# jamieapps101/Basic_Sparse_Matrix

Measured on AMD Instinct MI355X. Metric: CSR x dense SpMM effective GB/s (B_alg / step time); nnz/s, higher is better.
Workload: dtype f64

## Files before the change

### basic_sparse_matrix_amd/_lib.py

```python

from __future__ import annotations

import ctypes
import os
import threading

import numpy as np

try:
    import torch
except Exception:
    torch = None

LIB_PATH = os.environ.get("BSM_LIB_PATH") or os.path.join(os.path.dirname(os.path.abspath(__file__)), "lib",
                                                          "libbsm_hip.so")

BSM_F64, BSM_F32, BSM_I32, BSM_U32, BSM_I64, BSM_U64 = range(6)
DTYPE_CODES = {
    np.dtype(np.float64): BSM_F64,
    np.dtype(np.float32): BSM_F32,
    np.dtype(np.int32): BSM_I32,
    np.dtype(np.uint32): BSM_U32,
    np.dtype(np.int64): BSM_I64,
    np.dtype(np.uint64): BSM_U64,
}
CODE_DTYPES = {v: k for k, v in DTYPE_CODES.items()}

BSM_OK = 0
BSM_ERR_INVALID = 1
BSM_ERR_DIMENSIONS = 2
BSM_ERR_NON_SQUARE = 3
BSM_ERR_PANIC = 4
BSM_ERR_HIP = 5
BSM_ERR_OOM = 6
BSM_ERR_UNSUPPORTED = 7
BSM_TILED_ANY_PADDING = 1
BSM_ERR_NO_DEVICE = 8
BSM_ERR_OUT_OF_BOUNDS = 9
BSM_ERR_COMM = 10
BSM_UNIQUE_ID_BYTES = 128

ROWLEN_CONST, ROWLEN_UNIFORM, ROWLEN_BINOMIAL = 0, 1, 2
VAL_UNIFORM, VAL_SMALLINT = 0, 1


class DeviceUnavailable(RuntimeError):
    """The HIP library or a gfx950 device is not available (no CPU fallback)."""


class BsmError(RuntimeError):
    def __init__(self, code: int, msg: str):
        super().__init__(f"bsm error {code}: {msg}")
        self.code = code
        self.msg = msg


_u64 = ctypes.c_uint64
_u32 = ctypes.c_uint32
_int = ctypes.c_int
_vp = ctypes.c_void_p
_pp = ctypes.POINTER(ctypes.c_void_p)
_u64p = ctypes.POINTER(ctypes.c_uint64)

SIGNATURES = [
    ("bsm_api_version", _int, []),
    ("bsm_last_error", ctypes.c_char_p, []),
    ("bsm_stage_timing", _int, [_int]),
    ("bsm_stage_times", _int, [_int, ctypes.POINTER(_int), ctypes.c_char_p, ctypes.POINTER(ctypes.c_double)]),
    ("bsm_device_count", _int, [ctypes.POINTER(_int)]),
    ("bsm_set_device", _int, [_int]),
    ("bsm_csr_upload", _int, [_int, _u64, _u64, _u64, _vp, _vp, _vp, ctypes.POINTER(_vp)]),
    ("bsm_csr_from_inserts", _int, [_int, _u64, _u64, _u64, _vp, _vp, _vp, ctypes.POINTER(_vp)]),
    ("bsm_csr_from_coo", _int, [_int, _u64, _u64, _u64, _vp, _vp, _vp, ctypes.POINTER(_vp)]),
    ("bsm_csr_shape", _int, [_vp, _u64p, _u64p, _u64p, ctypes.POINTER(_int)]),
    ("bsm_csr_download", _int, [_vp, _vp, _vp, _vp]),
    ("bsm_host_register", _int, [_vp, _u64]),
    ("bsm_host_unregister", _int, [_vp]),
    ("bsm_csr_free", None, [_vp]),
    ("bsm_csr_mul_dense", _int, [_vp, _u64, _u64, _pp, ctypes.POINTER(_vp)]),
    ("bsm_csr_mul_vector", _int, [_vp, _vp, _u64, _vp, _u64]),
    ("bsm_csr_transpose", _int, [_vp, ctypes.POINTER(_vp)]),
    ("bsm_csr_add_sparse", _int, [_vp, _vp, ctypes.POINTER(_vp)]),
    ("bsm_csr_sub_sparse", _int, [_vp, _vp, ctypes.POINTER(_vp)]),
    ("bsm_csr_mul_sparse", _int, [_vp, _vp, ctypes.POINTER(_vp)]),
    ("bsm_csr_cholesky", _int, [_vp, ctypes.POINTER(_vp)]),
    ("bsm_forward_substitution", _int, [_vp, _u64, _u64, _pp, _pp]),
    ("bsm_backward_substitution", _int, [_vp, _u64, _u64, _pp, _pp]),
    ("bsm_solve", _int, [_vp, _u64, _u64, _pp, _pp]),
    ("bsm_solve_blocked", _int, [_vp, _u64, _u64, _pp, _pp]),
    ("bsm_solve_nd", _int, [_vp, _u64, _u64, _pp, _pp]),
    ("bsm_nd_factor_create", _int, [_vp, ctypes.POINTER(_vp)]),
    ("bsm_nd_factor_solve", _int, [_vp, _u64, _u64, _pp, _pp]),
    ("bsm_nd_factor_info", _int, [_vp, _u64p, ctypes.POINTER(_int), _u64p, _u64p]),
    ("bsm_nd_factor_perm", _int, [_vp, _vp]),
    ("bsm_nd_factor_export", _int, [_vp, ctypes.POINTER(_vp), ctypes.POINTER(_vp)]),
    ("bsm_nd_factor_refactor", _int, [_vp, _vp]),
    ("bsm_nd_factor_logdet", _int, [_vp, ctypes.POINTER(ctypes.c_double)]),
    ("bsm_nd_factor_solve_system", _int, [_vp, _int, _u64, _u64, _pp, _pp]),
    ("bsm_dev_nd_factor_solve", _int, [_vp, _int, _u64, _vp, _vp, _vp]),
    ("bsm_nd_factor_selinv", _int, [_vp, _vp, _u64, _vp, _vp, _vp]),
    ("bsm_dev_nd_factor_inv_diag", _int, [_vp, _vp, _vp]),
    ("bsm_nd_factor_free", None, [_vp]),
    ("bsm_nd_analyse", _int, [_u64, _vp, _vp, _u64, _vp, _vp, _u64, _u64p, _vp, _u64, _u64p]),
    ("bsm_nd_cache_clear", _int, []),
    ("bsm_nd_cache_info", _int, [_u64p, _u64p, _u64p, _u64p]),
    ("bsm_dev_gen_row_ptr", _int, [_u64, _u64, _u64, _u32, _int, _u32, _u32, _vp, _vp, _u64, _vp]),
    ("bsm_dev_gen_entries", _int, [_int, _u64, _u64, _u64, _u32, _int, _vp, _vp, _vp, _vp]),
    ("bsm_dev_gen_dense", _int, [_int, _u64, _u64, _u64, _u64, _int, _vp, _vp]),
    ("bsm_dev_gen_insert_stream", _int, [_int, _u64, _u64, _u64, _u64, _u64, _u64, _vp, _vp, _vp, _vp]),
    ("bsm_dev_csr_from_inserts", _int, [_int, _u64, _u64, _u64, _vp, _vp, _vp, ctypes.POINTER(_vp), _vp]),
    ("bsm_dev_scan_workspace_bytes", _u64, [_u64]),
    ("bsm_dev_spmm", _int, [_int, _u64, _u64, _u64, _vp, _vp, _vp, _u64, _vp, _vp, _vp, _vp]),
    ("bsm_csr_panel_cols", _int, [_vp, _u64p]),
    ("bsm_dev_spmm_panel_cols", _u64, [_int, _u64, _u64]),
    ("bsm_dev_spmm_plan_bytes", _u64, [_u64, _u64, _u64]),
    ("bsm_dev_spmm_plan", _int, [_u64, _u64, _vp, _vp, _u64, _vp, ctypes.POINTER(_int), _vp]),
    ("bsm_dev_spmm_panelled", _int, [_int, _u64, _u64, _u64, _vp, _vp, _vp, _u64, _vp, _vp, _vp, _u64, _vp, _vp]),
    ("bsm_dev_tiled_wanted", _int, [_int, _u64, _u64, _u64, _u64, _u64]),
    ("bsm_dev_tiled_create", _int, [_u64, _u64, _u64, _vp, _vp, _vp, _u64, _int, ctypes.POINTER(_vp), _vp]),
    ("bsm_dev_spmm_tiled", _int, [_vp, _vp, _vp, _vp, _vp]),
    ("bsm_tiled_info", _int, [_vp, _u64p, _u64p, _u64p]),
    ("bsm_tiled_destroy", None, [_vp]),
    ("bsm_csr_tiled", _int, [_vp, ctypes.POINTER(_int)]),
    ("bsm_dev_compact", _int, [_int, _u64, _u64, _vp, _vp, _vp, _vp, _vp, _vp, _u64, _vp]),
    ("bsm_multi_create", _int, [_int, ctypes.POINTER(_int), ctypes.POINTER(_vp)]),
    ("bsm_multi_unique_id", _int, [_vp]),
    ("bsm_multi_create_rank", _int, [_vp, _int, _int, _int, ctypes.POINTER(_vp)]),
    ("bsm_multi_create_external", _int, [_int, _int, _int, ctypes.POINTER(_vp)]),
    ("bsm_multi_is_external", _int, [_vp, ctypes.POINTER(_int)]),
    ("bsm_partition_rows", _int, [_vp, _u64, _u32, _vp]),
    ("bsm_multi_info", _int, [_vp, ctypes.POINTER(_int), ctypes.POINTER(_int), ctypes.POINTER(_int)]),
    ("bsm_multi_broadcast", _int, [_vp, _pp, _u64, _int]),
    ("bsm_multi_destroy", None, [_vp]),
    ("bsm_mcsr_upload", _int, [_vp, _int, _u64, _u64, _u64, _vp, _vp, _vp, _u32, ctypes.POINTER(_vp)]),
    ("bsm_mcsr_generate", _int, [_vp, _int, _u64, _u64, _u32, _int, _u32, _u32, _int, _u32, ctypes.POINTER(_vp)]),
    ("bsm_mcsr_info", _int, [_vp, _u64p, _u64p, _u64p, ctypes.POINTER(_u32), _u64p, _vp]),
    ("bsm_mcsr_prepare", _int, [_vp, _u64, _int, ctypes.POINTER(ctypes.c_double)]),
    ("bsm_mcsr_plan_info", _int, [_vp, ctypes.POINTER(_int), ctypes.POINTER(_int), _u64p, _u64p]),
    ("bsm_mcsr_mul_dense", _int, [_vp, _u64, _u64, _pp, ctypes.POINTER(_vp)]),
    ("bsm_mcsr_step", _int, [_vp, _pp]),
    ("bsm_mcsr_sync", _int, [_vp]),
    ("bsm_mcsr_step_times", _int, [_vp, _int, _int, ctypes.POINTER(_int), ctypes.POINTER(ctypes.c_double)]),
    ("bsm_mcsr_reset_times", None, [_vp]),
    ("bsm_mcsr_copy_y", _int, [_vp, _int, _vp, _vp]),
    ("bsm_mcsr_output", _int, [_vp, ctypes.POINTER(_vp)]),
    ("bsm_mcsr_compact", _int, [_vp]),
    ("bsm_mcsr_set_output_rank", _int, [_vp, _int]),
    ("bsm_mcsr_slot_read", _int, [_vp, _int, _u32, _u32, _vp, _vp]),
    ("bsm_mcsr_slot_write", _int, [_vp, _int, _u32, _u32, _vp, _vp]),
    ("bsm_mcsr_free", None, [_vp]),
]

_lock = threading.Lock()
_lib = None


def load(path: str = LIB_PATH) -> ctypes.CDLL:
    global _lib
    with _lock:
        if _lib is not None:
            return _lib
        if not os.path.exists(path):
            raise DeviceUnavailable(
                f"{path} is missing: build it with `python -c 'import __graft_entry__ as g; g.build()'`"
            )
        lib = ctypes.CDLL(path)
        for name, res, args in SIGNATURES:
            fn = getattr(lib, name)
            fn.restype = res
            fn.argtypes = args
        _lib = lib
        return lib


def stage_timing(on: bool = True) -> None:
    check(load().bsm_stage_timing(1 if on else 0))
# ... 138 lines not shown
```

### basic_sparse_matrix_amd/csrc/capi.hip

```cpp
#include <atomic>
#include <cstdarg>
#include <cstdlib>
#include <mutex>
#include <vector>

#include <algorithm>
#include <cstring>

#include "bsm_internal.hpp"

namespace bsm {

static thread_local std::string g_err;

void set_error(const char* fmt, ...) {
    char buf[1024];
    va_list ap;
    va_start(ap, fmt);
    vsnprintf(buf, sizeof(buf), fmt, ap);
    va_end(ap);
    g_err = buf;
}
const char* last_error() { return g_err.c_str(); }

// ... 1142 lines not shown
}

uint64_t bsm_dev_spmm_panel_cols(int dtype, uint64_t n_cols, uint64_t k) {
    return spmm_panel_cols(dtype, n_cols, k);
}

uint64_t bsm_dev_spmm_plan_bytes(uint64_t rows, uint64_t n_cols, uint64_t panel_cols) {
    return spmm_plan_bytes(rows, n_cols, panel_cols);
}

int bsm_dev_spmm_plan(uint64_t rows, uint64_t n_cols, const int64_t* row_ptr, const int32_t* col,
                      uint64_t panel_cols, int32_t* seg, int* usable, void* stream) {
    BSM_REQUIRE(row_ptr && usable && (spmm_plan_bytes(rows, n_cols, panel_cols) == 0 || seg),
                BSM_ERR_INVALID, "null argument");
    return spmm_plan(rows, n_cols, row_ptr, col, panel_cols, seg, usable,
                     static_cast<hipStream_t>(stream));
}

int bsm_dev_spmm_panelled(int dtype, uint64_t rows, uint64_t n_cols, uint64_t nnz,
                          const int64_t* row_ptr, const int32_t* col, const void* vals, uint64_t k,
                          const void* x, void* y, int32_t* row_nnz, uint64_t panel_cols,
                          const int32_t* seg, void* stream) {
    BSM_REQUIRE(row_ptr && (nnz == 0 || (col && vals)) && (k == 0 || (x && y)), BSM_ERR_INVALID,
                "null argument");
    if (k == 0) return BSM_OK;
    return spmm_panelled(dtype, rows, n_cols, nnz, row_ptr, col, vals, k, x, y, row_nnz, panel_cols,
                         seg, static_cast<hipStream_t>(stream));
}

int bsm_dev_tiled_wanted(int dtype, uint64_t rows, uint64_t n_cols, uint64_t nnz, uint64_t k,
                         uint64_t max_row_len) {
    return tiled_wanted(dtype, rows, n_cols, nnz, k, max_row_len) ? 1 : 0;
}

int bsm_dev_tiled_create(uint64_t rows, uint64_t n_cols, uint64_t nnz, const int64_t* row_ptr,
                         const int32_t* col, const double* vals, uint64_t k, int flags, bsm_tiled** out,
                         void* stream) {
    return tiled_create(BSM_F64, rows, n_cols, nnz, row_ptr, col, vals, k, flags, out, static_cast<hipStream_t>(stream));
}

int bsm_dev_spmm_tiled(const bsm_tiled* t, const double* x, double* y, int32_t* row_nnz, void* stream) {
    return tiled_spmm(t, x, y, row_nnz, false, static_cast<hipStream_t>(stream));
}

int bsm_tiled_info(const bsm_tiled* t, uint64_t* bytes, uint64_t* slots, uint64_t* panel_cols) {
    BSM_REQUIRE(t, BSM_ERR_INVALID, "null argument");
    const uint64_t n = (t->chunks + t->overread) * 64;
    if (bytes) *bytes = n * (t->meta_bytes + (t->dtype == BSM_F32 ? 4 : 8)) + ((uint64_t)t->nw * t->nb + 1) * 8;
    if (slots) *slots = t->chunks * 64;
    if (panel_cols) *panel_cols = 1ull << t->pshift;
    return BSM_OK;
}

void bsm_tiled_destroy(bsm_tiled* t) { tiled_destroy(t); }

int bsm_csr_tiled(const bsm_csr* m, int* in_use) {
    BSM_REQUIRE(m && in_use, BSM_ERR_INVALID, "null argument");
    std::lock_guard<std::mutex> lock(m->plan_mu);
    *in_use = m->tiled ? 1 : 0;
    return BSM_OK;
}

int bsm_dev_compact(int dtype, uint64_t rows, uint64_t k, const void* y, const int32_t* row_nnz,
                    int64_t* out_row_ptr, int32_t* out_col, void* out_vals, void* workspace,
                    uint64_t workspace_bytes, void* stream) {
    BSM_REQUIRE(row_nnz && out_row_ptr, BSM_ERR_INVALID, "null argument");
    hipStream_t s = static_cast<hipStream_t>(stream);
    BSM_TRY(exclusive_scan_i32_to_i64(row_nnz, out_row_ptr, rows, workspace, workspace_bytes, s));
    return compact_dispatch(dtype, rows, k, y, out_row_ptr, out_col, out_vals, s);
}

}
```

### basic_sparse_matrix_amd/csrc/kernels_tiled.hip

```cpp
#include "bsm_internal.hpp"

#include <cstdlib>
#include <type_traits>
#include <utility>
#include <vector>


namespace bsm {
namespace {

constexpr int WAVE = 64;
constexpr int CHUNK = 64;
constexpr int PHASES = 6;
constexpr int OVERREAD = 4;
constexpr uint32_t DONE = 0xffffffffu;
constexpr uint32_t RW_MAX = 155;
constexpr uint32_t RW_MAX_F32 = 255;
constexpr uint32_t PSHIFT = 12;
constexpr uint32_t PACE_PCT = 3;

__device__ __forceinline__ uint64_t lanemask_lt(int lane) {
    return lane == 0 ? 0ull : (~0ull >> (64 - lane));
}
__device__ __forceinline__ uint32_t wave_min_u32(uint32_t v) {
#pragma unroll
    for (int off = 1; off < WAVE; off <<= 1) v = min(v, (uint32_t)__shfl_xor((int)v, off, WAVE));
    return v;
}

template <bool WRITE, int SLOTS, typename V, typename M = uint32_t>
__global__ __launch_bounds__(256) void tiled_layout(uint64_t rows, uint64_t n_cols, double pace, uint32_t rbits,
                                                    uint32_t pad, const int64_t* __restrict__ rp,
                                                    const int32_t* __restrict__ col,
                                                    const V* __restrict__ vals, uint32_t nw,
                                                    uint32_t rpw, uint32_t nb, uint32_t rw, uint32_t pshift,
                                                    int32_t* __restrict__ counts,
                                                    const int64_t* __restrict__ offs,
                                                    M* __restrict__ meta, V* __restrict__ val) {
    const int lane = threadIdx.x & (WAVE - 1);
    const uint64_t task = (uint64_t)blockIdx.x * (blockDim.x / WAVE) + threadIdx.x / WAVE;
    if (task >= (uint64_t)nw * nb) return;
    const uint64_t gw = task / nb, b = task % nb;
    const uint64_t w0 = gw * rpw;
    const uint64_t wend = min<uint64_t>(rows, w0 + rpw);
    const uint64_t r0 = w0 + b * rw;
    int64_t cur[SLOTS], end[SLOTS];
    uint32_t h[SLOTS];
#pragma unroll
    for (int j = 0; j < SLOTS; ++j) {
        const uint32_t s = lane + WAVE * j;
        const bool live = s < rw && r0 + s < wend;
        cur[j] = live ? rp[r0 + s] : 0;
        end[j] = live ? rp[r0 + s + 1] : 0;
        h[j] = cur[j] < end[j] ? (uint32_t)col[cur[j]] >> pshift : DONE;
    }
    const bool any = r0 < wend;
    const int64_t t0 = any ? rp[r0] : 0, t1 = any ? rp[min<uint64_t>(r0 + rw, wend)] : 0;
    const double np = (double)(((n_cols - 1) >> pshift) + 1);
    const double inv_r = t1 > t0 ? (double)CHUNK * np / ((double)(t1 - t0) * pace) : 1e30;
    int64_t c = WRITE ? offs[task] : 0;
    int64_t n = 0;
    for (;;) {
        bool sel[SLOTS];
        int pos[SLOTS];
#pragma unroll
        for (int j = 0; j < SLOTS; ++j) {
            sel[j] = false;
            pos[j] = 0;
        }
        int taken = 0;
        const double pm = (double)n * inv_r;
        const uint32_t pmax = pm >= 4.0e9 ? DONE - 1 : (uint32_t)pm;
        bool done = false;
        while (taken < CHUNK) {
            uint32_t m = DONE;
#pragma unroll
            for (int j = 0; j < SLOTS; ++j) m = min(m, sel[j] ? DONE : h[j]);
            m = wave_min_u32(m);
            if (m == DONE) {
                done = taken == 0;
                break;
            }
            if (m > pmax) break;
            int before = 0;
#pragma unroll
            for (int j = 0; j < SLOTS; ++j) {
                const bool cand = !sel[j] && h[j] == m;
                const uint64_t bal = __ballot(cand);
                const int rank = before + __popcll(bal & lanemask_lt(lane));
                if (cand && taken + rank < CHUNK) {
                    sel[j] = true;
                    pos[j] = taken + rank;
                }
                before += __popcll(bal);
            }
            taken = min(taken + before, CHUNK);
        }
        if (done) break;
#pragma unroll
        for (int j = 0; j < SLOTS; ++j) {
            if (sel[j]) {
                const int64_t e = cur[j];
                if (WRITE) {
                    meta[c * CHUNK + pos[j]] = ((M)(uint32_t)col[e] << rbits) | (M)(lane + WAVE * j);
                    val[c * CHUNK + pos[j]] = vals[e];
                }
                cur[j] = e + 1;
                h[j] = cur[j] < end[j] ? (uint32_t)col[cur[j]] >> pshift : DONE;
            }
        }
        if (WRITE && lane >= taken) {
            meta[c * CHUNK + lane] = (M)rw;
            val[c * CHUNK + lane] = (V)0;
        }
        ++c;
        ++n;
    }
    const int64_t padded = (n + pad - 1) / pad * pad;
    if (WRITE) {
        for (int64_t p = n; p < padded; ++p, ++c) {
            meta[c * CHUNK + lane] = (M)rw;
            val[c * CHUNK + lane] = (V)0;
        }
    } else if (lane == 0) {
        counts[task] = (int32_t)padded;
    }
}

template <typename T> struct Vec2;
template <> struct Vec2<double> { using type = double2; };
struct F2 {
    uint64_t u;
};
template <> struct Vec2<float> { using type = F2; };
__device__ __forceinline__ double lo_of(const double2& v) { return v.x; }
__device__ __forceinline__ double hi_of(const double2& v) { return v.y; }
__device__ __forceinline__ float lo_of(const F2& v) { return __uint_as_float((uint32_t)v.u); }
__device__ __forceinline__ float hi_of(const F2& v) { return __uint_as_float((uint32_t)(v.u >> 32)); }
__device__ __forceinline__ double2 make_v2(double a, double b) { return make_double2(a, b); }
__device__ __forceinline__ F2 make_v2(float a, float b) {
    return F2{((uint64_t)__float_as_uint(b) << 32) | (uint64_t)__float_as_uint(a)};
}
template <typename T> using vec2_t = typename Vec2<T>::type;

template <typename T = double, typename M = uint32_t>
struct Idx {
    M mi;
    T vi;
};
template <typename T, typename M>
__device__ __forceinline__ void load_idx(Idx<T, M>& c, const M* __restrict__ meta, const T* __restrict__ val,
                                         int64_t chunk, int lane) {
    c.mi = meta[chunk * CHUNK + lane];
    c.vi = val[chunk * CHUNK + lane];
}
template <int I, typename T>
__device__ __forceinline__ uint32_t bm(const Idx<T, uint32_t>& c) {
    return (uint32_t)__builtin_amdgcn_update_dpp(0, (int)c.mi, 0x150 + I, 0xf, 0xf, false);
}
template <int I, typename T>
__device__ __forceinline__ uint64_t bm(const Idx<T, uint64_t>& c) {
    const uint32_t lo = (uint32_t)__builtin_amdgcn_update_dpp(0, (int)(uint32_t)c.mi, 0x150 + I, 0xf, 0xf, false);
// ... 259 lines not shown
    BSM_REQUIRE(k == 32 || k == 1, BSM_ERR_UNSUPPORTED, "tiled: k must be 32 or 1");
    BSM_REQUIRE(dtype == BSM_F64 || dtype == BSM_F32, BSM_ERR_UNSUPPORTED, "tiled: f64 or f32 only");
    const bool f32 = dtype == BSM_F32;
    const size_t es = f32 ? 4 : 8;
    const bool wide = k == 32 && n_cols >= (1ull << 24);
    const size_t mb = wide ? 8 : 4;
    const uint32_t rbits = k == 1 ? K1_RBITS : 8;
    BSM_REQUIRE(k == 32 ? n_cols <= 0x7fffffffull : n_cols < (1ull << (32 - rbits)), BSM_ERR_UNSUPPORTED,
                "tiled: columns must be < 2^%u", k == 32 ? 31u : 32 - rbits);
    *out = nullptr;
    int dev = 0;
    BSM_TRY(current_device(&dev));
    int cus = 0;
    BSM_HIP_TRY(hipDeviceGetAttribute(&cus, hipDeviceAttributeMultiprocessorCount, dev));
    if (s && cus > 0) {
        std::vector<uint32_t> mk((size_t)(cus + 31) / 32, 0u);
        if (hipExtStreamGetCUMask(s, (uint32_t)mk.size(), mk.data()) == hipSuccess) {
            int n = 0;
            for (int i = 0; i < cus; ++i) n += (mk[i / 32] >> (i % 32)) & 1u;
            if (n > 0 && n < cus) cus = n;
        } else {
            (void)hipGetLastError();
        }
    }
    const uint32_t wpc = k == 1 ? K1_WAVES_PER_CU : 4u;
    const uint32_t nw_env = env_u32("BSM_TILED_WAVES", wpc * (uint32_t)cus);
    const uint32_t nw = nw_env;
    const uint32_t k1_stage = env_u32("BSM_TILED_K1_STAGE", K1_STAGE_DEFAULT) == 8 ? 8u : 4u;
    const uint32_t rw_cap =
        k == 1 ? K1_RW_MAX : (f32 ? RW_MAX_F32 : RW_MAX);
    uint32_t rw_max = env_u32("BSM_TILED_RW", rw_cap);
    rw_max = rw_max < 8u ? 8u : (rw_max > rw_cap ? rw_cap : rw_max);
    const uint32_t pshift = env_u32("BSM_TILED_PSHIFT", k == 1 ? K1_PSHIFT : PSHIFT);
    const double pace = 1.0 + env_u32("BSM_TILED_PACE_PCT", PACE_PCT) / 100.0;
    const uint32_t pad = k == 1 ? 1u : PHASES;
    const uint32_t overread = k == 1 ? 2 * k1_stage : OVERREAD;
    BSM_REQUIRE(nw >= wpc && nw % wpc == 0 && pshift < 32, BSM_ERR_INVALID, "tiled: bad geometry");
    const uint64_t rpw64 = (rows + nw - 1) / nw;
    BSM_REQUIRE(rpw64 < (1ull << 31), BSM_ERR_UNSUPPORTED, "tiled: too many rows per wave");
    const uint32_t rpw = rpw64 ? (uint32_t)rpw64 : 1u;
    const uint32_t nb = (rpw + rw_max - 1) / rw_max;
    const uint32_t rw = (rpw + nb - 1) / nb;
    const uint64_t tasks = (uint64_t)nw * nb;

    DBuf counts, offs, ws;
    BSM_TRY(counts.alloc(tasks * sizeof(int32_t)));
    BSM_TRY(offs.alloc((tasks + 1) * sizeof(int64_t)));
    const uint64_t grid = (tasks + 3) / 4;
    auto layout = [&](auto write_tag, int32_t* cnt, const int64_t* of, void* me, void* va) -> int {
        constexpr bool W = decltype(write_tag)::value;
        auto go = [&]<typename V, typename MT>(V*, MT*) {
            if (k == 1)
                tiled_layout<W, (K1_RW_MAX + 1) / WAVE, V, MT><<<dim3((unsigned)grid), 256, 0, s>>>(
                    rows, n_cols, pace, rbits, pad, rp, col, static_cast<const V*>(vals), nw, rpw, nb, rw, pshift,
                    cnt, of, static_cast<MT*>(me), static_cast<V*>(va));
            else if (rw_cap > 192)
                tiled_layout<W, 4, V, MT><<<dim3((unsigned)grid), 256, 0, s>>>(
                    rows, n_cols, pace, rbits, pad, rp, col, static_cast<const V*>(vals), nw, rpw, nb, rw, pshift,
                    cnt, of, static_cast<MT*>(me), static_cast<V*>(va));
            else
                tiled_layout<W, 3, V, MT><<<dim3((unsigned)grid), 256, 0, s>>>(
                    rows, n_cols, pace, rbits, pad, rp, col, static_cast<const V*>(vals), nw, rpw, nb, rw, pshift,
                    cnt, of, static_cast<MT*>(me), static_cast<V*>(va));
        };
        if (f32 && wide) go((float*)nullptr, (uint64_t*)nullptr);
        else if (f32) go((float*)nullptr, (uint32_t*)nullptr);
        else if (wide) go((double*)nullptr, (uint64_t*)nullptr);
        else go((double*)nullptr, (uint32_t*)nullptr);
        BSM_HIP_TRY(hipGetLastError());
        return BSM_OK;
    };
    auto t_phase = host_now();
    auto phase_end = [&](double* acc) -> int {
        if (!pt) return BSM_OK;
        BSM_HIP_TRY(hipStreamSynchronize(s));
        *acc += ms_since(t_phase);
        t_phase = host_now();
        return BSM_OK;
    };
    BSM_TRY(layout(std::false_type{}, counts.as<int32_t>(), nullptr, nullptr, nullptr));
    BSM_TRY(phase_end(pt ? &pt->count_ms : nullptr));
    const uint64_t wsb = scan_workspace_bytes(tasks);
    BSM_TRY(ws.alloc(wsb));
    BSM_TRY(exclusive_scan_i32_to_i64(counts.as<int32_t>(), offs.as<int64_t>(), tasks, ws.p, wsb, s));
    int64_t total = 0;
    BSM_HIP_TRY(read_dev(&total, offs.as<int64_t>() + tasks, sizeof(total), s));
    BSM_TRY(phase_end(pt ? &pt->scan_ms : nullptr));
    BSM_REQUIRE((flags & BSM_TILED_ANY_PADDING) ||
                    (uint64_t)total * CHUNK <= nnz + nnz / 4 + tasks * pad * CHUNK + (uint64_t)CHUNK * 64,
                BSM_ERR_UNSUPPORTED, "tiled: %lld chunks for %llu entries (rows too uneven)", (long long)total,
                (unsigned long long)nnz);
    const uint64_t slots = ((uint64_t)total + overread) * CHUNK;
    size_t free_b = 0, total_b = 0;
    BSM_HIP_TRY(hipMemGetInfo(&free_b, &total_b));
    BSM_REQUIRE(slots * (mb + es) + (256ull << 20) + reserve < free_b, BSM_ERR_OOM,
                "tiled: %llu MB stream (+%llu MB reserved) does not fit", (unsigned long long)(slots * (mb + es) >> 20),
                (unsigned long long)(reserve >> 20));
    DBuf meta, val, bar;
    BSM_TRY(bar.alloc(8 * BAR_STRIDE * sizeof(unsigned)));
    BSM_TRY(meta.alloc(slots * mb));
    BSM_TRY(val.alloc(slots * es));
    BSM_TRY(phase_end(pt ? &pt->alloc_ms : nullptr));
    BSM_TRY(layout(std::true_type{}, nullptr, offs.as<int64_t>(), meta.p, val.p));
    BSM_HIP_TRY(hipMemsetAsync(static_cast<char*>(meta.p) + (uint64_t)total * CHUNK * mb, 0, overread * CHUNK * mb, s));
    BSM_HIP_TRY(hipMemsetAsync(static_cast<char*>(val.p) + (uint64_t)total * CHUNK * es, 0, overread * CHUNK * es, s));
    BSM_HIP_TRY(hipStreamSynchronize(s));
    BSM_TRY(phase_end(pt ? &pt->write_ms : nullptr));
    auto* t = new bsm_tiled;
    t->device = dev;
    t->dtype = dtype;
    t->k = k;
    t->rows = rows;
    t->n_cols = n_cols;
    t->nnz = nnz;
    t->nw = nw;
// ... 85 lines not shown
```

### basic_sparse_matrix_amd/device.py

```python

from __future__ import annotations

import ctypes
from dataclasses import dataclass

import numpy as np
import torch

from . import _lib

TORCH_DT = {
    np.dtype(np.float64): torch.float64,
    np.dtype(np.float32): torch.float32,
    np.dtype(np.int32): torch.int32,
    np.dtype(np.uint32): torch.uint32,
    np.dtype(np.int64): torch.int64,
    np.dtype(np.uint64): torch.uint64,
}


def _stream(stream=None) -> int:
    s = stream if stream is not None else torch.cuda.current_stream()
    return s.cuda_stream

# ... 53 lines not shown
            self.panel_cols, self.seg = w, seg
        return self.panel_cols

    def plan_tiled(self, k: int, force: bool = False) -> "TiledPlan | None":
        lib = _lib.require_device()
        self.tiled = None
        if self.dtype != np.float64 or k not in (1, 32) or self.nnz == 0:
            return None
        if not force:
            max_len = int((self.row_ptr[1:] - self.row_ptr[:-1]).max().item()) if self.rows else 0
            if not lib.bsm_dev_tiled_wanted(_lib.DTYPE_CODES[self.dtype], self.rows, self.n_cols, self.nnz, k,
                                            max_len):
                return None
        h = ctypes.c_void_p()
        rc = lib.bsm_dev_tiled_create(self.rows, self.n_cols, self.nnz, _p(self.row_ptr), _p(self.col),
                                      _p(self.vals), k, _lib.BSM_TILED_ANY_PADDING if force else 0,
                                      ctypes.byref(h), _stream())
        if rc in (_lib.BSM_ERR_UNSUPPORTED, _lib.BSM_ERR_OOM):
            return None
        _lib.check(rc)
        self.tiled = TiledPlan(h.value, k)
        return self.tiled

    def spmm(self, x: torch.Tensor, y: torch.Tensor, row_nnz: torch.Tensor | None = None, stream=None) -> None:
        lib = _lib.load()
        k = x.shape[1] if x.dim() == 2 else 1
        if self.tiled is not None and k == self.tiled.k:
            _lib.check(lib.bsm_dev_spmm_tiled(self.tiled.handle, _p(x), _p(y),
                                              _p(row_nnz) if row_nnz is not None else 0, _stream(stream)))
            return
        if self.seg is not None:
            _lib.check(lib.bsm_dev_spmm_panelled(_lib.DTYPE_CODES[self.dtype], self.rows, self.n_cols, self.nnz,
                                                 _p(self.row_ptr), _p(self.col), _p(self.vals), k, _p(x), _p(y),
                                                 _p(row_nnz) if row_nnz is not None else 0, self.panel_cols,
                                                 _p(self.seg), _stream(stream)))
            return
        _lib.check(lib.bsm_dev_spmm(_lib.DTYPE_CODES[self.dtype], self.rows, self.n_cols, self.nnz, _p(self.row_ptr),
                                    _p(self.col), _p(self.vals), k, _p(x), _p(y),
                                    _p(row_nnz) if row_nnz is not None else 0, _stream(stream)))


class TiledPlan:

    def __init__(self, handle: int, k: int = 32):
        self.handle = handle
        self.k = k

    def info(self) -> dict:
        lib = _lib.load()
        b, sl, pc = ctypes.c_uint64(), ctypes.c_uint64(), ctypes.c_uint64()
        _lib.check(lib.bsm_tiled_info(self.handle, ctypes.byref(b), ctypes.byref(sl), ctypes.byref(pc)))
        return {"bytes": b.value, "slots": sl.value, "panel_cols": pc.value}

    def __del__(self):
        if getattr(self, "handle", None) and _lib._lib is not None:
            _lib._lib.bsm_tiled_destroy(self.handle)
            self.handle = None


def gen_dense(seed, row0, n, k, value_kind=_lib.VAL_UNIFORM, dtype=np.float64, device="cuda") -> torch.Tensor:
    lib = _lib.require_device()
    dt = np.dtype(dtype)
    x = torch.empty((n, k), dtype=TORCH_DT[dt], device=device)
    _lib.check(lib.bsm_dev_gen_dense(_lib.DTYPE_CODES[dt], seed, row0, n, k, value_kind, _p(x), _stream()))
    return x


def nd_factor_solve(factor, b: torch.Tensor, out: torch.Tensor | None = None, *, system: str = "A",
                    stream=None) -> torch.Tensor:
    from .solver import nd_system_code
    from .sparse import _raise_for

    code = nd_system_code(system)
    want = TORCH_DT[np.dtype(factor.dtype)]
    out = torch.empty_like(b) if out is None else out
    for name, t in (("b", b), ("out", out)):
        if t.dtype != want:
            raise TypeError(f"nd_factor_solve: {name} is {t.dtype}, the factor is {factor.dtype}")
        if not t.is_cuda:
            raise ValueError(f"nd_factor_solve: {name} is not on the device")
        if t.dim() not in (1, 2) or t.shape[0] != factor.n or not t.is_contiguous():
            raise ValueError(f"nd_factor_solve: {name} must be contiguous, ({factor.n},) or ({factor.n}, k), "
                             f"got {tuple(t.shape)}")
    if out.shape != b.shape or out.device != b.device:
        raise ValueError(f"nd_factor_solve: out is {tuple(out.shape)} on {out.device}, b {tuple(b.shape)} on {b.device}")
    k = b.shape[1] if b.dim() == 2 else 1
    _raise_for(_lib.require_device().bsm_dev_nd_factor_solve(factor._h(), code, k, _p(b), _p(out), _stream(stream)))
    return out


def nd_factor_inv_diag(factor, out: torch.Tensor | None = None, *, stream=None) -> torch.Tensor:
    from .sparse import _raise_for

    h = factor._h()
    want = TORCH_DT[np.dtype(factor.dtype)]
    out = torch.empty((factor.n,), dtype=want, device="cuda") if out is None else out
    if out.dtype != want:
        raise TypeError(f"nd_factor_inv_diag: out is {out.dtype}, the factor is {factor.dtype}")
    if not out.is_cuda:
        raise ValueError("nd_factor_inv_diag: out is not on the device")
    if out.dim() != 1 or out.shape[0] != factor.n or not out.is_contiguous():
        raise ValueError(f"nd_factor_inv_diag: out must be contiguous, ({factor.n},), got {tuple(out.shape)}")
    _raise_for(_lib.require_device().bsm_dev_nd_factor_inv_diag(h, _p(out), _stream(stream)))
    return out


class Compactor:

    def __init__(self, rows: int, k: int, dtype, device="cuda"):
        lib = _lib.load()
# ... 41 lines not shown
```

### include/bsm.h

```cpp
#ifndef BSM_H
#define BSM_H

#include <stdint.h>

#ifdef __cplusplus
extern "C" {
#endif

#define BSM_API_VERSION 1

typedef enum bsm_dtype {
    BSM_F64 = 0,
    BSM_F32 = 1,
    BSM_I32 = 2,
    BSM_U32 = 3,
    BSM_I64 = 4,
    BSM_U64 = 5
} bsm_dtype;

typedef enum bsm_status {
    BSM_OK = 0,
    BSM_ERR_INVALID = 1,
    BSM_ERR_DIMENSIONS = 2,
    BSM_ERR_NON_SQUARE = 3,
// ... 60 lines not shown
int bsm_nd_factor_export(const bsm_nd_factor* f, bsm_csr** l, bsm_csr** l_star);
int bsm_nd_factor_refactor(bsm_nd_factor* f, const bsm_csr* a);
int bsm_nd_factor_logdet(const bsm_nd_factor* f, double* logdet);
int bsm_nd_factor_solve_system(const bsm_nd_factor* f, int system, uint64_t k, uint64_t n,
                               const void* const* b_cols, void* const* x_cols);
int bsm_dev_nd_factor_solve(const bsm_nd_factor* f, int system, uint64_t k, const void* b, void* x,
                            void* stream);
int bsm_nd_factor_selinv(const bsm_nd_factor* f, void* diag, uint64_t nq, const uint64_t* rows,
                         const uint64_t* cols, void* vals);
int bsm_dev_nd_factor_inv_diag(const bsm_nd_factor* f, void* diag, void* stream);
void bsm_nd_factor_free(bsm_nd_factor* f);
int bsm_nd_cache_clear(void);
int bsm_nd_cache_info(uint64_t* entries, uint64_t* kept_bytes, uint64_t* hits, uint64_t* misses);
int bsm_nd_analyse(uint64_t n, const uint64_t* row_ptr, const uint64_t* col_idx, uint64_t leaf,
                   int64_t* perm, int64_t* nodes, uint64_t cap, uint64_t* n_nodes, int64_t* st,
                   uint64_t st_cap, uint64_t* st_len);

int bsm_dev_gen_row_ptr(uint64_t seed, uint64_t row0, uint64_t rows, uint32_t n_cols,
                        int rowlen_kind, uint32_t a, uint32_t b, int64_t* row_ptr,
                        void* workspace, uint64_t workspace_bytes, void* stream);
int bsm_dev_gen_entries(int dtype, uint64_t seed, uint64_t row0, uint64_t rows,
                        uint32_t n_cols, int value_kind, const int64_t* row_ptr,
                        int32_t* col, void* vals, void* stream);
int bsm_dev_gen_insert_stream(int dtype, uint64_t seed, uint64_t i0, uint64_t n, uint64_t rows,
                              uint64_t cols, uint64_t vmod, uint64_t* row, uint64_t* col, void* vals,
                              void* stream);
int bsm_dev_csr_from_inserts(int dtype, uint64_t rows, uint64_t cols, uint64_t n, const uint64_t* row,
                             const uint64_t* col, const void* vals, bsm_csr** out, void* stream);
int bsm_dev_gen_dense(int dtype, uint64_t seed, uint64_t row0, uint64_t n, uint64_t k,
                      int value_kind, void* x, void* stream);
uint64_t bsm_dev_scan_workspace_bytes(uint64_t n);
int bsm_dev_spmm(int dtype, uint64_t rows, uint64_t n_cols, uint64_t nnz,
                 const int64_t* row_ptr, const int32_t* col, const void* vals, uint64_t k,
                 const void* x, void* y, int32_t* row_nnz, void* stream);
int bsm_csr_panel_cols(const bsm_csr* m, uint64_t* panel_cols);
uint64_t bsm_dev_spmm_panel_cols(int dtype, uint64_t n_cols, uint64_t k);
uint64_t bsm_dev_spmm_plan_bytes(uint64_t rows, uint64_t n_cols, uint64_t panel_cols);
int bsm_dev_spmm_plan(uint64_t rows, uint64_t n_cols, const int64_t* row_ptr, const int32_t* col,
                      uint64_t panel_cols, int32_t* seg, int* usable, void* stream);
int bsm_dev_spmm_panelled(int dtype, uint64_t rows, uint64_t n_cols, uint64_t nnz,
                          const int64_t* row_ptr, const int32_t* col, const void* vals, uint64_t k,
                          const void* x, void* y, int32_t* row_nnz, uint64_t panel_cols,
                          const int32_t* seg, void* stream);
typedef struct bsm_tiled bsm_tiled;
#define BSM_TILED_ANY_PADDING 1
int bsm_dev_tiled_wanted(int dtype, uint64_t rows, uint64_t n_cols, uint64_t nnz, uint64_t k,
                         uint64_t max_row_len);
int bsm_dev_tiled_create(uint64_t rows, uint64_t n_cols, uint64_t nnz, const int64_t* row_ptr,
                         const int32_t* col, const double* vals, uint64_t k, int flags,
                         bsm_tiled** out, void* stream);
int bsm_dev_spmm_tiled(const bsm_tiled* t, const double* x, double* y, int32_t* row_nnz,
                       void* stream);
int bsm_tiled_info(const bsm_tiled* t, uint64_t* bytes, uint64_t* slots, uint64_t* panel_cols);
int bsm_csr_tiled(const bsm_csr* m, int* in_use);
void bsm_tiled_destroy(bsm_tiled* t);
int bsm_dev_compact(int dtype, uint64_t rows, uint64_t k, const void* y,
                    const int32_t* row_nnz, int64_t* out_row_ptr, int32_t* out_col,
                    void* out_vals, void* workspace, uint64_t workspace_bytes, void* stream);

typedef struct bsm_multi bsm_multi;
typedef struct bsm_mcsr bsm_mcsr;
#define BSM_UNIQUE_ID_BYTES 128
int bsm_multi_create(int n_gpus, const int* devices, bsm_multi** out);
int bsm_multi_unique_id(void* id);
int bsm_multi_create_rank(const void* id, int world, int rank, int device, bsm_multi** out);
int bsm_multi_create_external(int world, int rank, int device, bsm_multi** out);
int bsm_multi_is_external(const bsm_multi* ctx, int* external);
int bsm_partition_rows(const uint64_t* row_ptr, uint64_t rows, uint32_t pieces, uint64_t* bounds);
int bsm_multi_info(const bsm_multi* ctx, int* world, int* n_local, int* first_rank);
int bsm_multi_broadcast(bsm_multi* ctx, void* const* bufs, uint64_t bytes, int root);
void bsm_multi_destroy(bsm_multi* ctx);

int bsm_mcsr_upload(bsm_multi* ctx, int dtype, uint64_t rows, uint64_t cols, uint64_t nnz,
                    const uint64_t* row_ptr, const uint64_t* col_idx, const void* vals, uint32_t chunks,
                    bsm_mcsr** out);
int bsm_mcsr_generate(bsm_multi* ctx, int dtype, uint64_t seed, uint64_t rows, uint32_t n_cols, int rowlen_kind,
                      uint32_t a, uint32_t b, int value_kind, uint32_t chunks, bsm_mcsr** out);
int bsm_mcsr_info(const bsm_mcsr* m, uint64_t* rows, uint64_t* cols, uint64_t* nnz, uint32_t* pieces,
                  uint64_t* piece_rows, uint64_t* bounds);
int bsm_mcsr_prepare(bsm_mcsr* m, uint64_t k, int schedule, double* plan_ms);
int bsm_mcsr_plan_info(const bsm_mcsr* m, int* tiled_pieces, int* local_pieces, uint64_t* copy_bytes,
                       uint64_t* panel_cols);
int bsm_mcsr_mul_dense(bsm_mcsr* m, uint64_t k, uint64_t x_rows, const void* const* x_cols, bsm_csr** out);
int bsm_mcsr_step(bsm_mcsr* m, const void* const* x_dev);
int bsm_mcsr_sync(bsm_mcsr* m);
int bsm_mcsr_step_times(bsm_mcsr* m, int local, int max, int* n, double* ms);
void bsm_mcsr_reset_times(bsm_mcsr* m);
int bsm_mcsr_copy_y(const bsm_mcsr* m, int local, void* y, int32_t* row_nnz);
int bsm_mcsr_output(const bsm_mcsr* m, bsm_csr** out);
int bsm_mcsr_set_output_rank(bsm_mcsr* m, int rank);
int bsm_mcsr_compact(bsm_mcsr* m);
int bsm_mcsr_slot_read(const bsm_mcsr* m, int local, uint32_t first, uint32_t n, void* y, int32_t* row_nnz);
int bsm_mcsr_slot_write(bsm_mcsr* m, int local, uint32_t first, uint32_t n, const void* y, const int32_t* row_nnz);
void bsm_mcsr_free(bsm_mcsr* m);

#ifdef __cplusplus
}
#endif

#endif
```

Before: 698.2.

## Speed up tiled layout build with DPP wave-min and windowed vector loads

The tiled_layout kernel that builds the tiled SpMM format now does its wave-wide minimum with DPP row operations plus readlane instead of a shuffle-xor loop. For small slot counts it also reads column indices and values through 32-byte aligned vector windows kept in registers, rather than issuing a scalar global load per element. The selection loop is rewritten to be branch-free. New geometry and download APIs expose the tiled buffers, presumably for verification. The cost is more register pressure from the per-slot windows, and the change only helps if layout construction falls inside the timed step.

```diff
diff --git a/basic_sparse_matrix_amd/_lib.py b/basic_sparse_matrix_amd/_lib.py
--- a/basic_sparse_matrix_amd/_lib.py
+++ b/basic_sparse_matrix_amd/_lib.py
@@ -61,6 +61,7 @@
 _vp = ctypes.c_void_p
 _pp = ctypes.POINTER(ctypes.c_void_p)
 _u64p = ctypes.POINTER(ctypes.c_uint64)
+_u32p = ctypes.POINTER(ctypes.c_uint32)
 
 SIGNATURES = [
     ("bsm_api_version", _int, []),
@@ -120,8 +121,11 @@
     ("bsm_dev_tiled_create", _int, [_u64, _u64, _u64, _vp, _vp, _vp, _u64, _int, ctypes.POINTER(_vp), _vp]),
     ("bsm_dev_spmm_tiled", _int, [_vp, _vp, _vp, _vp, _vp]),
     ("bsm_tiled_info", _int, [_vp, _u64p, _u64p, _u64p]),
+    ("bsm_tiled_geometry", _int, [_vp, _u64p, _u64p, _u32p, _u32p, _u32p, _u32p]),
+    ("bsm_tiled_download", _int, [_vp, _vp, _vp, _vp]),
     ("bsm_tiled_destroy", None, [_vp]),
     ("bsm_csr_tiled", _int, [_vp, ctypes.POINTER(_int)]),
+    ("bsm_csr_tiled_copy", _int, [_vp, ctypes.POINTER(_vp)]),
     ("bsm_dev_compact", _int, [_int, _u64, _u64, _vp, _vp, _vp, _vp, _vp, _vp, _u64, _vp]),
     ("bsm_multi_create", _int, [_int, ctypes.POINTER(_int), ctypes.POINTER(_vp)]),
     ("bsm_multi_unique_id", _int, [_vp]),
diff --git a/basic_sparse_matrix_amd/csrc/capi.hip b/basic_sparse_matrix_amd/csrc/capi.hip
--- a/basic_sparse_matrix_amd/csrc/capi.hip
+++ b/basic_sparse_matrix_amd/csrc/capi.hip
@@ -1218,12 +1218,40 @@
     return BSM_OK;
 }
 
+int bsm_tiled_geometry(const bsm_tiled* t, uint64_t* tasks, uint64_t* chunks, uint32_t* overread,
+                       uint32_t* meta_bytes, uint32_t* val_bytes, uint32_t* rw) {
+    BSM_REQUIRE(t, BSM_ERR_INVALID, "null argument");
+    if (tasks) *tasks = (uint64_t)t->nw * t->nb;
+    if (chunks) *chunks = t->chunks;
+    if (overread) *overread = t->overread;
+    if (meta_bytes) *meta_bytes = t->meta_bytes;
+    if (val_bytes) *val_bytes = t->dtype == BSM_F32 ? 4 : 8;
+    if (rw) *rw = t->rw;
+    return BSM_OK;
+}
+
+int bsm_tiled_download(const bsm_tiled* t, int64_t* offs, void* meta, void* val) {
+    BSM_REQUIRE(t, BSM_ERR_INVALID, "null argument");
+    const uint64_t n = (t->chunks + t->overread) * 64;
+    if (offs) BSM_HIP_TRY(hipMemcpy(offs, t->offs, ((uint64_t)t->nw * t->nb + 1) * sizeof(int64_t), hipMemcpyDeviceToHost));
+    if (meta) BSM_HIP_TRY(hipMemcpy(meta, t->meta, n * t->meta_bytes, hipMemcpyDeviceToHost));
+    if (val) BSM_HIP_TRY(hipMemcpy(val, t->val, n * (t->dtype == BSM_F32 ? 4 : 8), hipMemcpyDeviceToHost));
+    return BSM_OK;
+}
+
 void bsm_tiled_destroy(bsm_tiled* t) { tiled_destroy(t); }
 
 int bsm_csr_tiled(const bsm_csr* m, int* in_use) {
     BSM_REQUIRE(m && in_use, BSM_ERR_INVALID, "null argument");
     std::lock_guard<std::mutex> lock(m->plan_mu);
     *in_use = m->tiled ? 1 : 0;
+    return BSM_OK;
+}
+
+int bsm_csr_tiled_copy(const bsm_csr* m, const bsm_tiled** out) {
+    BSM_REQUIRE(m && out, BSM_ERR_INVALID, "null argument");
+    std::lock_guard<std::mutex> lock(m->plan_mu);
+    *out = m->tiled;
     return BSM_OK;
 }
 
diff --git a/basic_sparse_matrix_amd/csrc/kernels_tiled.hip b/basic_sparse_matrix_amd/csrc/kernels_tiled.hip
--- a/basic_sparse_matrix_amd/csrc/kernels_tiled.hip
+++ b/basic_sparse_matrix_amd/csrc/kernels_tiled.hip
@@ -22,21 +22,73 @@
 __device__ __forceinline__ uint64_t lanemask_lt(int lane) {
     return lane == 0 ? 0ull : (~0ull >> (64 - lane));
 }
+template <int CTRL, int ROW_MASK>
+__device__ __forceinline__ uint32_t dpp_min_u32(uint32_t v) {
+    return min(v, (uint32_t)__builtin_amdgcn_update_dpp((int)DONE, (int)v, CTRL, ROW_MASK, 0xf, false));
+}
 __device__ __forceinline__ uint32_t wave_min_u32(uint32_t v) {
-#pragma unroll
-    for (int off = 1; off < WAVE; off <<= 1) v = min(v, (uint32_t)__shfl_xor((int)v, off, WAVE));
-    return v;
+    v = dpp_min_u32<0x111, 0xf>(v);
+    v = dpp_min_u32<0x112, 0xf>(v);
+    v = dpp_min_u32<0x114, 0xf>(v);
+    v = dpp_min_u32<0x118, 0xf>(v);
+    v = dpp_min_u32<0x142, 0xa>(v);
+    v = dpp_min_u32<0x143, 0xc>(v);
+    return (uint32_t)__builtin_amdgcn_readlane((int)v, WAVE - 1);
+}
+
+constexpr int WIN_BYTES = 32;
+template <typename T>
+struct alignas(16) Vec16 {
+    T v[16 / sizeof(T)];
+};
+template <typename T>
+__device__ __forceinline__ uint32_t win_mis(const T* a) {
+    return (uint32_t)(reinterpret_cast<uintptr_t>(a) / sizeof(T)) & (WIN_BYTES / sizeof(T) - 1);
+}
+template <typename T, int N>
+__device__ __forceinline__ void win_load(T (&w)[N], const T* __restrict__ a, uint32_t mis, int64_t e, int64_t n) {
+    static_assert(N * sizeof(T) == WIN_BYTES);
+    constexpr int PER = 16 / sizeof(T);
+    const int64_t e0 = ((e + mis) & ~(int64_t)(N - 1)) - mis;
+    if (e0 >= 0 && e0 + N <= n) {
+        const Vec16<T>* p = reinterpret_cast<const Vec16<T>*>(a + e0);
+#pragma unroll
+        for (int i = 0; i < N / PER; ++i) {
+            const Vec16<T> q = p[i];
+#pragma unroll
+            for (int u = 0; u < PER; ++u) w[i * PER + u] = q.v[u];
+        }
+    } else {
+#pragma unroll
+        for (int i = 0; i < N; ++i) w[i] = (e0 + i >= 0 && e0 + i < n) ? a[e0 + i] : (T)0;
+    }
+}
+template <typename T, int N>
+__device__ __forceinline__ T win_pick_n(const T* w, uint32_t i) {
+    if constexpr (N == 1) {
+        return w[0];
+    } else {
+        const T lo = win_pick_n<T, N / 2>(w, i), hi = win_pick_n<T, N / 2>(w + N / 2, i);
+        return (i & (N / 2)) ? hi : lo;
+    }
+}
+template <typename T, int N>
+__device__ __forceinline__ T win_pick(const T (&w)[N], uint32_t i) {
+    return win_pick_n<T, N>(w, i);
 }
 
 template <bool WRITE, int SLOTS, typename V, typename M = uint32_t>
-__global__ __launch_bounds__(256) void tiled_layout(uint64_t rows, uint64_t n_cols, double pace, uint32_t rbits,
-                                                    uint32_t pad, const int64_t* __restrict__ rp,
+__global__ __launch_bounds__(256) void tiled_layout(uint64_t rows, uint64_t n_cols, int64_t nnz, double pace,
+                                                    uint32_t rbits, uint32_t pad, const int64_t* __restrict__ rp,
                                                     const int32_t* __restrict__ col,
                                                     const V* __restrict__ vals, uint32_t nw,
                                                     uint32_t rpw, uint32_t nb, uint32_t rw, uint32_t pshift,
                                                     int32_t* __restrict__ counts,
                                                     const int64_t* __restrict__ offs,
                                                     M* __restrict__ meta, V* __restrict__ val) {
+    constexpr bool WIN = SLOTS <= 4;
+    constexpr int WC = WIN ? WIN_BYTES / (int)sizeof(int32_t) : 1;
+    constexpr int WV = WIN && WRITE ? WIN_BYTES / (int)sizeof(V) : 1;
     const int lane = threadIdx.x & (WAVE - 1);
     const uint64_t task = (uint64_t)blockIdx.x * (blockDim.x / WAVE) + threadIdx.x / WAVE;
     if (task >= (uint64_t)nw * nb) return;
@@ -44,16 +96,42 @@
     const uint64_t w0 = gw * rpw;
     const uint64_t wend = min<uint64_t>(rows, w0 + rpw);
     const uint64_t r0 = w0 + b * rw;
+    const uint32_t cmis = WIN ? win_mis(col) : 0, vmis = WIN && WRITE ? win_mis(vals) : 0;
     int64_t cur[SLOTS], end[SLOTS];
     uint32_t h[SLOTS];
+    uint32_t cc[SLOTS];
+    int32_t wc[SLOTS][WC];
+    V wv[SLOTS][WV];
+    auto refill = [&](int j, bool first) {
+        if constexpr (WIN) {
+            if (cur[j] < end[j]) {
+                if (first || ((uint32_t)(cur[j] + cmis) & (WC - 1)) == 0) win_load(wc[j], col, cmis, cur[j], nnz);
+                if constexpr (WRITE) {
+                    if (first || ((uint32_t)(cur[j] + vmis) & (WV - 1)) == 0) win_load(wv[j], vals, vmis, cur[j], nnz);
+                }
+            }
+        }
+    };
+    auto settle = [&](int j) {
+        if (cur[j] < end[j]) {
+            if constexpr (WIN) cc[j] = (uint32_t)win_pick(wc[j], (uint32_t)(cur[j] + cmis) & (WC - 1));
+            else cc[j] = (uint32_t)col[cur[j]];
+            h[j] = cc[j] >> pshift;
+        } else {
+            h[j] = DONE;
+        }
+    };
 #pragma unroll
     for (int j = 0; j < SLOTS; ++j) {
         const uint32_t s = lane + WAVE * j;
         const bool live = s < rw && r0 + s < wend;
         cur[j] = live ? rp[r0 + s] : 0;
         end[j] = live ? rp[r0 + s + 1] : 0;
-        h[j] = cur[j] < end[j] ? (uint32_t)col[cur[j]] >> pshift : DONE;
-    }
+        cc[j] = 0;
+        refill(j, true);
+    }
+#pragma unroll
+    for (int j = 0; j < SLOTS; ++j) settle(j);
     const bool any = r0 < wend;
     const int64_t t0 = any ? rp[r0] : 0, t1 = any ? rp[min<uint64_t>(r0 + rw, wend)] : 0;
     const double np = (double)(((n_cols - 1) >> pshift) + 1);
@@ -61,12 +139,12 @@
     int64_t c = WRITE ? offs[task] : 0;
     int64_t n = 0;
     for (;;) {
-        bool sel[SLOTS];
+        uint32_t hs[SLOTS];
         int pos[SLOTS];
 #pragma unroll
         for (int j = 0; j < SLOTS; ++j) {
-            sel[j] = false;
-            pos[j] = 0;
+            hs[j] = h[j];
+            pos[j] = -1;
         }
         int taken = 0;
         const double pm = (double)n * inv_r;
@@ -75,7 +153,7 @@
         while (taken < CHUNK) {
             uint32_t m = DONE;
 #pragma unroll
-            for (int j = 0; j < SLOTS; ++j) m = min(m, sel[j] ? DONE : h[j]);
+            for (int j = 0; j < SLOTS; ++j) m = min(m, hs[j]);
             m = wave_min_u32(m);
             if (m == DONE) {
                 done = taken == 0;
@@ -85,13 +163,12 @@
             int before = 0;
 #pragma unroll
             for (int j = 0; j < SLOTS; ++j) {
-                const bool cand = !sel[j] && h[j] == m;
+                const bool cand = hs[j] == m;
                 const uint64_t bal = __ballot(cand);
-                const int rank = before + __popcll(bal & lanemask_lt(lane));
-                if (cand && taken + rank < CHUNK) {
-                    sel[j] = true;
-                    pos[j] = taken + rank;
-                }
+                const int at = taken + before + __popcll(bal & lanemask_lt(lane));
+                const bool take = cand && at < CHUNK;
+                pos[j] = take ? at : pos[j];
+                hs[j] = take ? DONE : hs[j];
                 before += __popcll(bal);
             }
             taken = min(taken + before, CHUNK);
@@ -99,15 +176,20 @@
         if (done) break;
 #pragma unroll
         for (int j = 0; j < SLOTS; ++j) {
-            if (sel[j]) {
+            if (pos[j] >= 0) {
                 const int64_t e = cur[j];
-                if (WRITE) {
-                    meta[c * CHUNK + pos[j]] = ((M)(uint32_t)col[e] << rbits) | (M)(lane + WAVE * j);
-                    val[c * CHUNK + pos[j]] = vals[e];
+                if constexpr (WRITE) {
+                    meta[c * CHUNK + pos[j]] = ((M)cc[j] << rbits) | (M)(lane + WAVE * j);
+                    if constexpr (WIN) val[c * CHUNK + pos[j]] = win_pick(wv[j], (uint32_t)(e + vmis) & (WV - 1));
+                    else val[c * CHUNK + pos[j]] = vals[e];
                 }
                 cur[j] = e + 1;
-                h[j] = cur[j] < end[j] ? (uint32_t)col[cur[j]] >> pshift : DONE;
+                refill(j, false);
             }
+        }
+#pragma unroll
+        for (int j = 0; j < SLOTS; ++j) {
+            if (pos[j] >= 0) settle(j);
         }
         if (WRITE && lane >= taken) {
             meta[c * CHUNK + lane] = (M)rw;
@@ -473,15 +555,15 @@
         auto go = [&]<typename V, typename MT>(V*, MT*) {
             if (k == 1)
                 tiled_layout<W, (K1_RW_MAX + 1) / WAVE, V, MT><<<dim3((unsigned)grid), 256, 0, s>>>(
-                    rows, n_cols, pace, rbits, pad, rp, col, static_cast<const V*>(vals), nw, rpw, nb, rw, pshift,
+                    rows, n_cols, (int64_t)nnz, pace, rbits, pad, rp, col, static_cast<const V*>(vals), nw, rpw, nb, rw, pshift,
                     cnt, of, static_cast<MT*>(me), static_cast<V*>(va));
             else if (rw_cap > 192)
                 tiled_layout<W, 4, V, MT><<<dim3((unsigned)grid), 256, 0, s>>>(
-                    rows, n_cols, pace, rbits, pad, rp, col, static_cast<const V*>(vals), nw, rpw, nb, rw, pshift,
+                    rows, n_cols, (int64_t)nnz, pace, rbits, pad, rp, col, static_cast<const V*>(vals), nw, rpw, nb, rw, pshift,
                     cnt, of, static_cast<MT*>(me), static_cast<V*>(va));
             else
                 tiled_layout<W, 3, V, MT><<<dim3((unsigned)grid), 256, 0, s>>>(
-                    rows, n_cols, pace, rbits, pad, rp, col, static_cast<const V*>(vals), nw, rpw, nb, rw, pshift,
+                    rows, n_cols, (int64_t)nnz, pace, rbits, pad, rp, col, static_cast<const V*>(vals), nw, rpw, nb, rw, pshift,
                     cnt, of, static_cast<MT*>(me), static_cast<V*>(va));
         };
         if (f32 && wide) go((float*)nullptr, (uint64_t*)nullptr);
diff --git a/basic_sparse_matrix_amd/device.py b/basic_sparse_matrix_amd/device.py
--- a/basic_sparse_matrix_amd/device.py
+++ b/basic_sparse_matrix_amd/device.py
@@ -129,10 +129,28 @@
         _lib.check(lib.bsm_tiled_info(self.handle, ctypes.byref(b), ctypes.byref(sl), ctypes.byref(pc)))
         return {"bytes": b.value, "slots": sl.value, "panel_cols": pc.value}
 
+    def download(self) -> dict:
+        return tiled_download(self.handle)
+
     def __del__(self):
         if getattr(self, "handle", None) and _lib._lib is not None:
             _lib._lib.bsm_tiled_destroy(self.handle)
             self.handle = None
+
+
+def tiled_download(handle: int) -> dict:
+    lib = _lib.load()
+    tasks, chunks = ctypes.c_uint64(), ctypes.c_uint64()
+    over, mb, vb, rw = ctypes.c_uint32(), ctypes.c_uint32(), ctypes.c_uint32(), ctypes.c_uint32()
+    _lib.check(lib.bsm_tiled_geometry(handle, ctypes.byref(tasks), ctypes.byref(chunks), ctypes.byref(over),
+                                      ctypes.byref(mb), ctypes.byref(vb), ctypes.byref(rw)))
+    n = (chunks.value + over.value) * 64
+    offs = np.empty(tasks.value + 1, dtype=np.int64)
+    meta = np.empty(n, dtype=np.uint64 if mb.value == 8 else np.uint32)
+    val = np.empty(n, dtype=np.uint64 if vb.value == 8 else np.uint32)
+    _lib.check(lib.bsm_tiled_download(handle, offs.ctypes.data, meta.ctypes.data, val.ctypes.data))
+    return {"tasks": tasks.value, "chunks": chunks.value, "overread": over.value, "rw": rw.value,
+            "offs": offs, "meta": meta, "val": val}
 
 
 def gen_dense(seed, row0, n, k, value_kind=_lib.VAL_UNIFORM, dtype=np.float64, device="cuda") -> torch.Tensor:
diff --git a/include/bsm.h b/include/bsm.h
--- a/include/bsm.h
+++ b/include/bsm.h
@@ -136,7 +136,11 @@
 int bsm_dev_spmm_tiled(const bsm_tiled* t, const double* x, double* y, int32_t* row_nnz,
                        void* stream);
 int bsm_tiled_info(const bsm_tiled* t, uint64_t* bytes, uint64_t* slots, uint64_t* panel_cols);
+int bsm_tiled_geometry(const bsm_tiled* t, uint64_t* tasks, uint64_t* chunks, uint32_t* overread,
+                       uint32_t* meta_bytes, uint32_t* val_bytes, uint32_t* rw);
+int bsm_tiled_download(const bsm_tiled* t, int64_t* offs, void* meta, void* val);
 int bsm_csr_tiled(const bsm_csr* m, int* in_use);
+int bsm_csr_tiled_copy(const bsm_csr* m, const bsm_tiled** out);
 void bsm_tiled_destroy(bsm_tiled* t);
 int bsm_dev_compact(int dtype, uint64_t rows, uint64_t k, const void* y,
                     const int32_t* row_nnz, int64_t* out_row_ptr, int32_t* out_col,
```

New measurement: 685.5. 1.8% lower.
